# nv-nguyen/gigapose

Hardware: AMD Instinct MI355X
Metric: query-crops/sec (ViT feat + template NN + 4DoF regress), 162 templates, 1/2/4/8 GPU (higher is better)
Workload: dtype f32 (ViT linear layers + attention, matcher, IST convolutions: f32 operands split into f16 hi/lo, 3 x f16 MFMA per k-block, f32 accumulate -- error vs f64 below the f32 fmaf chain's, tests/test_gpu_split.py; everything else f32); 1 GPU; BASELINE configs[1]: dinov2_vitl14 random-init, 1 object(s) x 162 templates, batch=64 crops per GPU, k=5, full path ViT->match->IST->RANSAC->pose; numerics=split, global_batch=64, parallelism=single, streams=single stream, rccl_ranks=0

## Files before the change

gigapose_amd/csrc/gp_match.hip:

```cpp
#include "gp_common.h"

namespace {

__global__ __launch_bounds__(256) void l2norm_cp_kernel(const float* __restrict__ x,
                                                         float* __restrict__ out, int C)
{
    const size_t base = (size_t)blockIdx.x * C * GP_P + threadIdx.x;
    float ss = 0.f;
    for (int c = 0; c < C; ++c) {
        const float v = x[base + (size_t)c * GP_P];
        ss = __builtin_fmaf(v, v, ss);
    }
    const float d = fmaxf(__builtin_sqrtf(ss), 1e-12f);
    const int c0 = blockIdx.y * 32;
    for (int c = c0; c < c0 + 32 && c < C; ++c) out[base + (size_t)c * GP_P] = x[base + (size_t)c * GP_P] / d;
}

using MM = KMajor<4, 2, 2, 4, 16>;
static_assert(MM::BM == 256 && MM::BN == 256 && MM::NT == 512, "matcher tile must be 256x256");

struct alignas(16) MatchSmem {
    float stage[MM::LDS_FLOATS];
    float qmask[GP_P];
    float smask[GP_P];
// ... 471 lines not shown
        sm.smask_p[pidx] = 0.f;
        sm.s_of[pidx] = (short)kDeadPatch;
#pragma unroll
        for (int w = 0; w < 4; ++w) { sm.colv[w][pidx] = 0.f; sm.coli[w][pidx] = 0; }
    }
    __syncthreads();
    int rank = before;
    for (int w = 4 * grp; w < wave; ++w) rank += sm.cnt[w];
    if (live) {
        if (tid < GP_P) {
            sm.t_of[rank] = (short)pidx;
            sm.qmask_p[rank] = mv;
        } else {
            sm.s_of[rank] = (short)pidx;
            sm.smask_p[rank] = mv;
        }
    }
    __syncthreads();
    const int live_t = sm.cnt[0] + sm.cnt[1] + sm.cnt[2] + sm.cnt[3], live_s = sm.cnt[4] + sm.cnt[5] + sm.cnt[6] + sm.cnt[7];
    const int nrb = __builtin_amdgcn_readfirstlane((live_t + 31) >> 5), ncb = __builtin_amdgcn_readfirstlane((live_s + 31) >> 5);
    const MatchWaveTile wt = match_wave_tile_unpack((unsigned)__builtin_amdgcn_readfirstlane((int)kMatchRect[nrb][ncb][wave]));

    const unsigned plane_bytes = (unsigned)GP_P * (unsigned)C * 2u;
    MatchSplitRsrc rs;
    rs.qh = __builtin_amdgcn_make_buffer_rsrc((void*)(q_hi + (size_t)b * GP_P * C), 0, plane_bytes, 0x00020000);
    rs.ql = __builtin_amdgcn_make_buffer_rsrc((void*)(q_lo + (size_t)b * GP_P * C), 0, plane_bytes, 0x00020000);
    rs.bh = __builtin_amdgcn_make_buffer_rsrc((void*)(b_hi + on * GP_P * C), 0, plane_bytes, 0x00020000);
    rs.bl = __builtin_amdgcn_make_buffer_rsrc((void*)((BANK_LO ? b_lo : b_hi) + on * GP_P * C), 0, plane_bytes, 0x00020000);
    {
        const int r0 = tid >> 2, r1 = r0 + 128;
        const unsigned ck = (unsigned)(tid & 3) * 16u, rowb = (unsigned)C * 2u;
        const int t0 = sm.t_of[r0], t1 = sm.t_of[r1], s0 = sm.s_of[r0], s1 = sm.s_of[r1];
        rs.va0 = t0 != kDeadPatch ? (unsigned)t0 * rowb + ck : kMatchOob;
        rs.va1 = t1 != kDeadPatch ? (unsigned)t1 * rowb + ck : kMatchOob;
        rs.vb0 = s0 != kDeadPatch ? (unsigned)s0 * rowb + ck : kMatchOob;
        rs.vb1 = s1 != kDeadPatch ? (unsigned)s1 * rowb + ck : kMatchOob;
    }

    f32x16 acc[2][4];
#pragma unroll
    for (int mi = 0; mi < 2; ++mi)
#pragma unroll
        for (int ni = 0; ni < 4; ++ni)
#pragma unroll
            for (int r = 0; r < 16; ++r) acc[mi][ni][r] = 0.f;
    const int ns = C / MS_BK;
    if (TRACE && tid == 0) trace[1] = wall_clock64();
    if (nrb > 0 && ncb > 0) {
        const int sel = wt.mi_n * 8 + wt.ni_n;
#define M_CASE(MI_, NI_) case MI_ * 8 + NI_: match_split_kloop<BANK_LO, MI_, NI_>(sm, acc, rs, ns, tid, lane, wt.r0, wt.c0, grp); break
        switch (sel) {
            M_CASE(1, 1); M_CASE(1, 2); M_CASE(1, 3); M_CASE(1, 4);
            M_CASE(2, 1); M_CASE(2, 2); M_CASE(2, 3);
            default: match_split_kloop<BANK_LO, 2, 4>(sm, acc, rs, ns, tid, lane, wt.r0, wt.c0, grp); break;
        }
#undef M_CASE
    }
    __syncthreads();
    if (TRACE && tid == 0) trace[2] = wall_clock64();

    constexpr float inv = 1.0f / (kFeatScale * kFeatScale);
#pragma unroll
    for (int mi = 0; mi < 2; ++mi)
#pragma unroll
        for (int ni = 0; ni < 4; ++ni)
#pragma unroll
            for (int r = 0; r < 16; ++r) acc[mi][ni][r] *= inv;
    match_epilogue<true>(sm, acc, b, n, N, thr, patch_thr, idx_t2s, score_t2s, mask_all, sim_avg, trace, src2tar, compact, wt);
}

__global__ __launch_bounds__(256) void l2norm_split_kernel(const float* __restrict__ x, _Float16* __restrict__ hi,
                                                            _Float16* __restrict__ lo, int C, int Cp,
                                                            const float* __restrict__ mask_img = nullptr, int mh = 0, int mw = 0,
                                                            float* __restrict__ patch_mask = nullptr)
{
    __shared__ float t[32][GP_P + 1];
    __shared__ float dn[GP_P];
    const int row = blockIdx.x, p = threadIdx.x;
    if (patch_mask && blockIdx.y == 0)
        patch_mask[(size_t)row * GP_P + p] = mask_img[(size_t)row * mh * mw + (size_t)((p >> 4) * (mh / GP_G)) * mw + (p & 15) * (mw / GP_G)];
    const float* xr = x + (size_t)row * C * GP_P;
    float ss = 0.f;
    int c = 0;
    for (; c + 16 <= C; c += 16) {
        float v[16];
#pragma unroll
        for (int u = 0; u < 16; ++u) v[u] = xr[(size_t)(c + u) * GP_P + p];
#pragma unroll
        for (int u = 0; u < 16; ++u) ss = __builtin_fmaf(v[u], v[u], ss);
    }
    for (; c < C; ++c) {
        const float v = xr[(size_t)c * GP_P + p];
        ss = __builtin_fmaf(v, v, ss);
    }
    dn[p] = fmaxf(__builtin_sqrtf(ss), 1e-12f);
    const int ngrp = Cp / 32, g0 = ngrp * blockIdx.y / gridDim.y, g1 = ngrp * (blockIdx.y + 1) / gridDim.y;
    for (int grp = g0; grp < g1; ++grp) {
        const int c0 = grp * 32;
        __syncthreads();
        for (int r = 0; r < 32; ++r) t[r][p] = (c0 + r < C) ? xr[(size_t)(c0 + r) * GP_P + p] : 0.f;
        __syncthreads();
#pragma unroll
        for (int u = 0; u < 4; ++u) {
            const int item = p + 256 * u, pp = item >> 2, g = item & 3;
            h16x8 h, l;
#pragma unroll
            for (int e = 0; e < 8; ++e) {
                const float v = (t[g * 8 + e][pp] / dn[pp]) * kFeatScale;
                const _Float16 hh = (_Float16)v;
                h[e] = hh;
                l[e] = (_Float16)(v - (float)hh);
            }
            const size_t o = ((size_t)row * GP_P + pp) * Cp + c0 + g * 8;
            *reinterpret_cast<h16x8*>(hi + o) = h;
            *reinterpret_cast<h16x8*>(lo + o) = l;
        }
    }
}

__global__ __launch_bounds__(64) void topk_kernel(const float* __restrict__ sim_avg, int N, int k,
                                                   int* __restrict__ ids, float* __restrict__ scores)
{
    extern __shared__ unsigned char taken[];
    const int b = blockIdx.x, lane = threadIdx.x;
    for (int n = lane; n < N; n += 64) taken[n] = 0;
    __syncthreads();
    const float* v = sim_avg + (size_t)b * N;
    for (int j = 0; j < k; ++j) {
        float bv = 0.f;
        int bi = 0x7fffffff;
        for (int n = lane; n < N; n += 64) {
            if (taken[n]) continue;
            const float x = v[n];
            if (bi == 0x7fffffff || x > bv) { bv = x; bi = n; }
        }
#pragma unroll
        for (int off = 32; off >= 1; off >>= 1) {
            const float ov = __shfl_xor(bv, off);
            const int oi = __shfl_xor(bi, off);
            if (oi != 0x7fffffff && (bi == 0x7fffffff || ov > bv || (ov == bv && oi < bi))) { bv = ov; bi = oi; }
        }
        if (lane == 0) {
            ids[(size_t)b * k + j] = bi;
            scores[(size_t)b * k + j] = bv;
            taken[bi] = 1;
        }
        __syncthreads();
    }
}

__global__ __launch_bounds__(256) void gather_records_kernel(
    const int* __restrict__ ids, const uint8_t* __restrict__ idx_t2s,
    const float* __restrict__ score_t2s, const float* __restrict__ mask_all, int N, int k,
    uint8_t* __restrict__ rec_idx, float* __restrict__ rec_score, float* __restrict__ rec_mask)
{
    const int bk = blockIdx.x, b = bk / k, t = threadIdx.x;
    const size_t src = ((size_t)b * N + ids[bk]) * GP_P + t;
    const size_t dst = (size_t)bk * GP_P + t;
    rec_idx[dst] = idx_t2s[src];
    rec_score[dst] = score_t2s[src];
    rec_mask[dst] = mask_all[src];
}

__global__ __launch_bounds__(256) void format_points_kernel(const uint8_t* __restrict__ rec_idx,
                                                             const float* __restrict__ rec_mask,
                                                             long long* __restrict__ tar_pts,
                                                             long long* __restrict__ src_pts)
{
    const size_t i = (size_t)blockIdx.x * GP_P + threadIdx.x;
    const int t = threadIdx.x;
    const bool valid = rec_mask[i] != 0.f;
    const int js = rec_idx[i];
// ... 215 lines not shown
```

gigapose_amd/csrc/gp_vit.hip:

```cpp
#include "gp_common.h"

int gp_gemm_launch(const float* A, int lda, const float* B, int ldb, float* D, int ldd, int I, int J,
                   int K, int epilogue, const float* bias, const float* scale, const float* res, int ldr,
                   float* sk_ws, hipStream_t st);
int gp_gemm_split_launch(const float* act, int ld_act, const void* whi, const void* wlo, float* D, int ldd, int I, int J,
                         int K, int act_is_b, int epilogue, const float* bias, const float* scale, const float* res, int ldr,
                         hipStream_t st);
bool gp_gemm_split256_usable(int I, int J, int K);
int gp_gemm_split256_launch(const float* act, int ld_act, const void* whi, const void* wlo, float* D, int ldd, int I, int J,
                            int K, int act_is_b, int epilogue, const float* bias, const float* scale, const float* res, int ldr,
                            float* scratch, hipStream_t st);
size_t gp_gemm_streamk_bytes();
int gp_gemm_streamk_reset_launch(float* sk_ws, hipStream_t st);
bool gp_gemm_split256_usable(int I, int J, int K);
bool gp_gemm_planes256_usable(int I, int J, int J_valid, int K);
int gp_gemm_planes256_launch(const void* ahi, const void* alo, const void* bhi, const void* blo, float* D, int ldd, void* ohi,
                             void* olo, int ldo, int I, int J, int J_valid, int K, int epilogue, const float* bias, const float* scale,
                             const float* res, int ldr, float out_scale, float* scratch, hipStream_t st, unsigned long long* trace = nullptr,
                             const GpPlaneOut* po = nullptr);

namespace {

constexpr int PATCH = 14, IMG = 224, KPE = 588, KPE_PAD = 592, T_TOK = 257;

// ... 65 lines not shown

int launch_layernorm(const float* X, float* Y, const float* g, const float* b, int C, int Mpad, float eps,
                     hipStream_t st)
{
    GpProfScope prof(GP_PROF_LN, 8.0 * C * Mpad, st);
    hipLaunchKernelGGL(layernorm_wide_kernel, dim3(Mpad / 64), dim3(1024), 0, st, X, Y, g, b, C, Mpad, eps);
    return 0;
}


typedef _Float16 v16x8 __attribute__((ext_vector_type(8)));
typedef _Float16 v16x4 __attribute__((ext_vector_type(4)));
typedef unsigned int au32x4 __attribute__((ext_vector_type(4)));
typedef float f32x2 __attribute__((ext_vector_type(2)));
constexpr float kPlaneScale = 8.0f;

__global__ __launch_bounds__(1024) void layernorm_planes_kernel(const float* __restrict__ X, _Float16* __restrict__ Yhi,
                                                                 _Float16* __restrict__ Ylo, const float* __restrict__ gamma,
                                                                 const float* __restrict__ beta, int C, int Mpad, float eps,
                                                                 int* __restrict__ status, float plane_scale, float* __restrict__ amax)
{
    __shared__ float red[16][64];
    const int tok = threadIdx.x & 63, sl = threadIdx.x >> 6;
    const int per = C >> 4, c0 = sl * per;
    const float* x = X + (size_t)c0 * Mpad + (size_t)blockIdx.x * 64 + tok;
    int bad = 0;
    float vmax = 0.f;
    float s = 0.f;
#pragma unroll 8
    for (int i = 0; i < per; ++i) s += x[(size_t)i * Mpad];
    red[sl][tok] = s;
    __syncthreads();
    float tot = 0.f;
#pragma unroll
    for (int j = 0; j < 16; ++j) tot += red[j][tok];
    const float mean = tot / (float)C;
    __syncthreads();
    float q = 0.f;
#pragma unroll 8
    for (int i = 0; i < per; ++i) {
        const float d = x[(size_t)i * Mpad] - mean;
        q = __builtin_fmaf(d, d, q);
    }
    red[sl][tok] = q;
    __syncthreads();
    tot = 0.f;
#pragma unroll
    for (int j = 0; j < 16; ++j) tot += red[j][tok];
    const float rstd = 1.0f / __builtin_sqrtf(tot / (float)C + eps);
    __shared__ unsigned int tile[2][128 * 65];
    const float* xb = X + (size_t)blockIdx.x * 64 + tok;
    const int t2 = 8 * (sl & 7) + (tok & 7), g2 = 8 * (sl >> 3) + (tok >> 3);
    const size_t row = ((size_t)blockIdx.x * 64 + t2) * C + 8 * g2;
    const int nchunk = C >> 7;
    for (int k = 0; k < nchunk; ++k) {
        unsigned int* T = tile[k & 1];
#pragma unroll
        for (int e = 0; e < 8; ++e) {
            const int cl = 8 * sl + e, c = 128 * k + cl;
            const float y = (xb[(size_t)c * Mpad] - mean) * rstd * gamma[c] + beta[c];
            const float v = y * plane_scale;
            const _Float16 hh = (_Float16)v;
            const _Float16 ll = (_Float16)(v - (float)hh);
            bad |= !(fabsf(v) <= kSplitPlaneLimit);
            vmax = __builtin_elementwise_maximum(vmax, __builtin_fabsf(v));
            T[cl * 65 + tok] = (unsigned int)__builtin_bit_cast(unsigned short, hh) |
                               ((unsigned int)__builtin_bit_cast(unsigned short, ll) << 16);
        }
        __syncthreads();
        v16x8 h, l;
#pragma unroll
        for (int e = 0; e < 8; ++e) {
            const unsigned int w = T[(8 * g2 + e) * 65 + t2];
            h[e] = __builtin_bit_cast(_Float16, (unsigned short)(w & 0xffffu));
            l[e] = __builtin_bit_cast(_Float16, (unsigned short)(w >> 16));
        }
        *reinterpret_cast<v16x8*>(Yhi + row + 128 * k) = h;
        *reinterpret_cast<v16x8*>(Ylo + row + 128 * k) = l;
    }
    if (bad) gp_raise(status, GP_ST_SPLIT_RANGE);
    if (amax) gp_record_amax(amax, vmax, 1.0f / plane_scale);
}

template <int NK, int TOK = 32>
__global__ __launch_bounds__(512) void layernorm_planes_reg_kernel(const float* __restrict__ X, _Float16* __restrict__ Yhi,
                                                                    _Float16* __restrict__ Ylo, const float* __restrict__ gamma,
                                                                    const float* __restrict__ beta, int Mpad, float eps,
                                                                    int* __restrict__ status, float plane_scale, float* __restrict__ amax)
{
    constexpr int C = 128 * NK, SL = 512 / TOK, CH = 8 * SL, NC = C / CH;
    constexpr int TP = CH + 4;
    static_assert(C % CH == 0 && (TOK == 32 || TOK == 16), "layernorm_planes_reg_kernel: C must be a multiple of the chunk width");
    __shared__ float red[SL][TOK];
    __shared__ __attribute__((aligned(16))) unsigned int tile[2][TOK * TP];
    __shared__ __attribute__((aligned(16))) float gb[2][C];
    const int tok = threadIdx.x & (TOK - 1), sl = threadIdx.x / TOK;
    const size_t tok0 = (size_t)blockIdx.x * TOK;
    float xv[NC][8];
    float s = 0.f;
#pragma unroll
    for (int k = 0; k < NC; ++k)
#pragma unroll
        for (int e = 0; e < 8; ++e) {
            xv[k][e] = X[(size_t)(CH * k + 8 * sl + e) * Mpad + tok0 + tok];
            s += xv[k][e];
        }
    for (int c = threadIdx.x; c < C; c += 512) {
        gb[0][c] = gamma[c];
        gb[1][c] = beta[c];
    }
    red[sl][tok] = s;
    __syncthreads();
    float tot = 0.f;
#pragma unroll
    for (int j = 0; j < SL; ++j) tot += red[j][tok];
    const float mean = tot / (float)C;
    __syncthreads();
    float q = 0.f;
#pragma unroll
    for (int k = 0; k < NC; ++k)
#pragma unroll
        for (int e = 0; e < 8; ++e) {
            const float d = xv[k][e] - mean;
            q = __builtin_fmaf(d, d, q);
        }
    red[sl][tok] = q;
    __syncthreads();
    tot = 0.f;
#pragma unroll
    for (int j = 0; j < SL; ++j) tot += red[j][tok];
    const float rstd = 1.0f / __builtin_sqrtf(tot / (float)C + eps);
    const int g2 = threadIdx.x & (SL - 1), t2 = threadIdx.x / SL;
    const size_t row = (tok0 + t2) * C + 8 * g2;
    int bad = 0;
    float vmax = 0.f;
#pragma unroll
    for (int k = 0; k < NC; ++k) {
        unsigned int* T = tile[k & 1];
        const int c = CH * k + 8 * sl;
        const f32x4 g0 = *reinterpret_cast<const f32x4*>(gb[0] + c), g1 = *reinterpret_cast<const f32x4*>(gb[0] + c + 4);
        const f32x4 b0 = *reinterpret_cast<const f32x4*>(gb[1] + c), b1 = *reinterpret_cast<const f32x4*>(gb[1] + c + 4);
        unsigned int w[8];
#pragma unroll
        for (int e = 0; e < 8; ++e) {
            const float y = (xv[k][e] - mean) * rstd * (e < 4 ? g0[e] : g1[e - 4]) + (e < 4 ? b0[e] : b1[e - 4]);
            const float v = y * plane_scale;
            const _Float16 hh = (_Float16)v;
            const _Float16 ll = (_Float16)(v - (float)hh);
            bad |= !(fabsf(v) <= kSplitPlaneLimit);
            if (amax) vmax = __builtin_elementwise_maximum(vmax, __builtin_fabsf(v));
            w[e] = (unsigned int)__builtin_bit_cast(unsigned short, hh) | ((unsigned int)__builtin_bit_cast(unsigned short, ll) << 16);
        }
        typedef unsigned int u4 __attribute__((ext_vector_type(4)));
        u4 w0 = {w[0], w[1], w[2], w[3]}, w1 = {w[4], w[5], w[6], w[7]};
        *reinterpret_cast<u4*>(T + tok * TP + 8 * sl) = w0;
        *reinterpret_cast<u4*>(T + tok * TP + 8 * sl + 4) = w1;
        __syncthreads();
        const u4 r0 = *reinterpret_cast<const u4*>(T + t2 * TP + 8 * g2), r1 = *reinterpret_cast<const u4*>(T + t2 * TP + 8 * g2 + 4);
        v16x8 h, l;
#pragma unroll
        for (int e = 0; e < 4; ++e) {
            h[e] = __builtin_bit_cast(_Float16, (unsigned short)(r0[e] & 0xffffu));
            l[e] = __builtin_bit_cast(_Float16, (unsigned short)(r0[e] >> 16));
            h[4 + e] = __builtin_bit_cast(_Float16, (unsigned short)(r1[e] & 0xffffu));
            l[4 + e] = __builtin_bit_cast(_Float16, (unsigned short)(r1[e] >> 16));
        }
        *reinterpret_cast<v16x8*>(Yhi + row + CH * k) = h;
        *reinterpret_cast<v16x8*>(Ylo + row + CH * k) = l;
    }
    if (bad) gp_raise(status, GP_ST_SPLIT_RANGE);
    if (amax) gp_record_amax(amax, vmax, 1.0f / plane_scale);
}


static int g_ln_planes_reg = 1;
#ifdef GP_PROBES
extern "C" void gp_vit_set_ln_reg(int on) { g_ln_planes_reg = (on >= 0 && on <= 2) ? on : 1; }
#endif

int launch_layernorm_planes(const float* X, _Float16* hi, _Float16* lo, const float* g, const float* b, int C, int Mpad, float eps,
                            hipStream_t st, float plane_scale = kPlaneScale, float* amax = nullptr)
{
    GpProfScope prof(GP_PROF_LN, 8.0 * C * Mpad, st);
    if (g_ln_planes_reg && C == 1024 && Mpad % 32 == 0 && Mpad / 32 <= 128 && g_ln_planes_reg != 2)
        hipLaunchKernelGGL((layernorm_planes_reg_kernel<8, 16>), dim3(Mpad / 16), dim3(512), 0, st, X, hi, lo, g, b, Mpad, eps, gp_status_buffer(), plane_scale, amax);
    else if (g_ln_planes_reg && C == 1024 && Mpad % 32 == 0)
        hipLaunchKernelGGL(layernorm_planes_reg_kernel<8>, dim3(Mpad / 32), dim3(512), 0, st, X, hi, lo, g, b, Mpad, eps, gp_status_buffer(), plane_scale, amax);
    else if (g_ln_planes_reg && C == 768 && Mpad % 32 == 0)
        hipLaunchKernelGGL(layernorm_planes_reg_kernel<6>, dim3(Mpad / 32), dim3(512), 0, st, X, hi, lo, g, b, Mpad, eps, gp_status_buffer(), plane_scale, amax);
    else
        hipLaunchKernelGGL(layernorm_planes_kernel, dim3(Mpad / 64), dim3(1024), 0, st, X, hi, lo, g, b, C, Mpad, eps, gp_status_buffer(), plane_scale, amax);
    return 0;
}

constexpr int NKT = 9;

__device__ __forceinline__ void attention_body(const float* __restrict__ Qp, const float* __restrict__ Kp,
                                               const float* __restrict__ Vp, float* __restrict__ Op, int q0, int C,
                                               int Mpad, float scale)
{
    const int lane = threadIdx.x, half = lane >> 5, l31 = lane & 31;
    const int tq = q0 + l31;
    const int tq_c = tq < T_TOK ? tq : T_TOK - 1;
    f32x16 o0, o1;
#pragma unroll
    for (int r = 0; r < 16; ++r) { o0[r] = 0.f; o1[r] = 0.f; }
    float m_run = -INFINITY, l_part = 0.f;

#pragma unroll 1
    for (int ch = 0; ch < 3; ++ch) {
        f32x16 s[3];
        int tk_c[3];
#pragma unroll
        for (int t = 0; t < 3; ++t) {
#pragma unroll
            for (int r = 0; r < 16; ++r) s[t][r] = 0.f;
            const int tk = (ch * 3 + t) * 32 + l31;
            tk_c[t] = tk < T_TOK ? tk : T_TOK - 1;
        }
#pragma unroll 8
        for (int kk = 0; kk < 32; ++kk) {
            const size_t drow = (size_t)(2 * kk + half) * Mpad;
            const float qv = Qp[drow + tq_c];
#pragma unroll
            for (int t = 0; t < 3; ++t) {
                const float kv = Kp[drow + tk_c[t]];
                s[t] = __builtin_amdgcn_mfma_f32_32x32x2f32(kv, qv, s[t], 0, 0, 0);
            }
        }
        float cmax = -INFINITY;
#pragma unroll
        for (int t = 0; t < 3; ++t)
#pragma unroll
            for (int r = 0; r < 16; ++r) {
                const int tk = (ch * 3 + t) * 32 + frag_row(r, lane);
                const float v = (tk < T_TOK) ? s[t][r] * scale : -INFINITY;
                s[t][r] = v;
                cmax = fmaxf(cmax, v);
            }
        cmax = fmaxf(cmax, __shfl_xor(cmax, 32));
        const float m_new = fmaxf(m_run, cmax);
        const float alpha = expf(m_run - m_new);
        float psum = 0.f;
#pragma unroll
        for (int t = 0; t < 3; ++t)
#pragma unroll
            for (int r = 0; r < 16; ++r) {
                const float p = expf(s[t][r] - m_new);
                s[t][r] = p;
                psum += p;
            }
        l_part = l_part * alpha + psum;
#pragma unroll
        for (int r = 0; r < 16; ++r) { o0[r] *= alpha; o1[r] *= alpha; }
        m_run = m_new;
#pragma unroll
        for (int t = 0; t < 3; ++t)
#pragma unroll
            for (int r = 0; r < 16; ++r) {
                int tk = (ch * 3 + t) * 32 + frag_row(r, lane);
                tk = tk < T_TOK ? tk : T_TOK - 1;
                const float* vrow = Vp + (size_t)tk * C + l31;
                const float v0 = vrow[0], v1 = vrow[32];
                o0 = __builtin_amdgcn_mfma_f32_32x32x2f32(v0, s[t][r], o0, 0, 0, 0);
                o1 = __builtin_amdgcn_mfma_f32_32x32x2f32(v1, s[t][r], o1, 0, 0, 0);
            }
    }
    const float inv = 1.0f / (l_part + __shfl_xor(l_part, 32));
    if (tq < T_TOK) {
#pragma unroll
        for (int r = 0; r < 16; ++r) {
            const int d = frag_row(r, lane);
// ... 267 lines not shown
            const _Float16* kl = sKl + tid * AKS;
            float a = 0.f;
#pragma unroll
            for (int c8 = 0; c8 < 8; ++c8) {
                const v16x8 h8 = *reinterpret_cast<const v16x8*>(kh + 8 * c8), l8 = *reinterpret_cast<const v16x8*>(kl + 8 * c8);
#pragma unroll
                for (int e = 0; e < 8; ++e) {
                    a = __builtin_fmaf((float)h8[e], xq[8 * c8 + e], a);
                    a = __builtin_fmaf((float)l8[e], xq[8 * c8 + e], a);
                }
            }
            sv = a * (0.125f * inv_s2);
        }
        float mx = sv;
#pragma unroll
        for (int off = 32; off >= 1; off >>= 1) mx = fmaxf(mx, __shfl_xor(mx, off));
        if (lane == 0) xred[0][wave] = mx;
        __syncthreads();
        mx = xred[0][0];
#pragma unroll
        for (int w = 1; w < 8; ++w) mx = fmaxf(mx, xred[0][w]);
        const float pr = tid < T_TOK ? exp_neg(sv - mx) : 0.f;
        if (tid < T_TOK) xs[tid] = pr;
        float ps = pr;
#pragma unroll
        for (int off = 32; off >= 1; off >>= 1) ps += __shfl_xor(ps, off);
        if (lane == 0) xred[1][wave] = ps;
        __syncthreads();
        {
            const _Float16* vh = sVh + lane * AVS + 32 * wave;
            const _Float16* vl = sVl + lane * AVS + 32 * wave;
            v16x4 h4[8], l4[8];
            f32x4 p4[8];
#pragma unroll
            for (int u = 0; u < 8; ++u) {
                h4[u] = *reinterpret_cast<const v16x4*>(vh + 4 * u);
                l4[u] = *reinterpret_cast<const v16x4*>(vl + 4 * u);
                p4[u] = *reinterpret_cast<const f32x4*>(xs + 32 * wave + 4 * u);
            }
            float a = 0.f;
#pragma unroll
            for (int u = 0; u < 8; ++u)
#pragma unroll
                for (int e = 0; e < 4; ++e) {
                    a = __builtin_fmaf((float)h4[u][e], p4[u][e], a);
                    a = __builtin_fmaf((float)l4[u][e], p4[u][e], a);
                }
            if (wave == 0) {
                a = __builtin_fmaf((float)sVh[lane * AVS + T_TOK - 1], xs[T_TOK - 1], a);
                a = __builtin_fmaf((float)sVl[lane * AVS + T_TOK - 1], xs[T_TOK - 1], a);
            }
            xo[wave][lane] = a;
        }
        __syncthreads();
        if (tid < 64) {
            float l = xred[1][0], a = xo[0][tid];
#pragma unroll
            for (int w = 1; w < 8; ++w) { l += xred[1][w]; a += xo[w][tid]; }
            float v = a * (1.0f / l);
            asm volatile("" : "+v"(v));
            const _Float16 hh = (_Float16)v;
            const size_t o = (tok0 + (T_TOK - 1)) * C + h * 64 + tid;
            Ohi[o] = hh;
            Olo[o] = (_Float16)(v - (float)hh);
        }
    }
}

static bool g_vit_planes = true;
#ifdef GP_PROBES
extern "C" void gp_vit_set_planes(int on) { g_vit_planes = on != 0; }
#endif

__global__ __launch_bounds__(256) void features_kernel(const float* __restrict__ X, float* __restrict__ out,
                                                        int C, int Mpad, int normalize, int* __restrict__ status)
{
    const int b = blockIdx.x, p = threadIdx.x;
    const int c0 = (int)((long long)C * blockIdx.y / gridDim.y), c1 = (int)((long long)C * (blockIdx.y + 1) / gridDim.y);
    const float* x = X + (size_t)b * T_TOK + 1 + p;
    float d = 1.f;
    if (normalize) {
        float ss = 0.f;
        int c = 0;
        for (; c + 16 <= C; c += 16) {
            float v[16];
#pragma unroll
            for (int u = 0; u < 16; ++u) v[u] = x[(size_t)(c + u) * Mpad];
#pragma unroll
            for (int u = 0; u < 16; ++u) ss = __builtin_fmaf(v[u], v[u], ss);
        }
        for (; c < C; ++c) {
            const float v = x[(size_t)c * Mpad];
            ss = __builtin_fmaf(v, v, ss);
        }
        d = fmaxf(__builtin_sqrtf(ss), 1e-12f);
        if (blockIdx.y == 0 && !(ss <= 3.0e38f)) gp_raise(status, GP_ST_SPLIT_RANGE);
    }
    float* o = out + (size_t)b * C * GP_P + p;
    for (int c = c0; c < c1; ++c) o[(size_t)c * GP_P] = normalize ? x[(size_t)c * Mpad] / d : x[(size_t)c * Mpad];
}

int launch_features(const float* X, float* out, int B, int C, int Mpad, int normalize, hipStream_t st)
{
    hipLaunchKernelGGL(features_kernel, dim3(B, B >= 64 ? 4 : (B >= 16 ? 16 : 32)), dim3(256), 0, st, X, out, C, Mpad, normalize,
                       gp_status_buffer());
    return 0;
}

inline int round_up(int x, int m) { return (x + m - 1) / m * m; }

}

enum { W_PATCH_WT = 0, W_PATCH_B, W_CLS_POS, W_POS_T, W_HEADER = 4 };
enum { L_LN1_G = 0, L_LN1_B, L_QK_WT, L_QK_B, L_V_WT, L_V_B, L_PROJ_WT, L_PROJ_B, L_LS1, L_LN2_G, L_LN2_B,
       L_FC1_WT, L_FC1_B, L_FC2_WT, L_FC2_B, L_LS2, L_PER_LAYER = 16 };

extern "C" {

size_t gp_vit_workspace_bytes(int B, int dim, int mlp_dim)
{
    if (B <= 0 || dim <= 0 || mlp_dim <= 0) return 0;
    const size_t Mpad = (size_t)round_up(B * T_TOK, 256);
    size_t f = (size_t)mlp_dim * Mpad;
    const size_t pe_need = (size_t)KPE_PAD * B * GP_P + (size_t)dim * B * GP_P;
    if (pe_need > f) f = pe_need;
    return sizeof(float) * ((size_t)5 * dim * Mpad + f) + gp_gemm_streamk_bytes();
}

enum { S_QK_HI = 0, S_QK_LO, S_V_HI, S_V_LO, S_PROJ_HI, S_PROJ_LO, S_FC1_HI, S_FC1_LO, S_FC2_HI, S_FC2_LO, S_PER_LAYER = 10 };
int gp_vit_forward_split2(const float* images, int B, int dim, int depth, int heads, int mlp_dim, float ln_eps,
                          const float* const* weights, int n_weights, const void* const* split, int n_split,
                          float* workspace, size_t workspace_bytes, float* out_features, int normalize,
                          int stop_after_layers, const float* plane_scales, float* plane_amax, void* stream);

int gp_attention_split_scaled(const void* qkv_hi, const void* qkv_lo, void* out_hi, void* out_lo, int B, int heads, int dim, int Mpad,
                              float qkv_scale, void* stream);
int gp_attention_split_scaled(const void* qkv_hi, const void* qkv_lo, void* out_hi, void* out_lo, int B, int heads, int dim, int Mpad,
                              float qkv_scale, void* stream)
{
    GP_REQUIRE(qkv_scale > 0.f, "gp_attention_split: bad plane scale");
    GP_REQUIRE(qkv_hi && qkv_lo && out_hi && out_lo && B > 0 && heads > 0 && dim == heads * 64 && Mpad >= B * T_TOK,
               "gp_attention_split: bad arguments");
    hipLaunchKernelGGL(attention_split_kernel, dim3(xcd_chunked_grid(B * heads)), dim3(ATH), 0, (hipStream_t)stream,
                       (const _Float16*)qkv_hi, (const _Float16*)qkv_lo, (_Float16*)out_hi, (_Float16*)out_lo, B, heads, dim, Mpad, 1.0f / (qkv_scale * qkv_scale));
    GP_CHECK_LAUNCH("gp_attention_split");
    return GP_OK;
}

int gp_layernorm_planes(const float* X, void* out_hi, void* out_lo, const float* gamma, const float* beta, int C, int Mpad, float eps,
                        void* stream)
{
    GP_REQUIRE(X && out_hi && out_lo && gamma && beta && C > 0 && C % 128 == 0 && Mpad > 0 && Mpad % 64 == 0, "gp_layernorm_planes: bad arguments");
    launch_layernorm_planes(X, (_Float16*)out_hi, (_Float16*)out_lo, gamma, beta, C, Mpad, eps, (hipStream_t)stream);
    GP_CHECK_LAUNCH("gp_layernorm_planes");
    return GP_OK;
}

#ifdef GP_PROBES
int gp_vit_attention_f32(const float* qk, const float* vt, float* out, int B, int heads, int dim, int Mpad, void* stream)
{
    GP_REQUIRE(qk && vt && out && B > 0 && heads > 0 && dim == heads * 64 && Mpad > 0 && Mpad % 256 == 0 && (long long)Mpad >= (long long)B * T_TOK,
               "gp_vit_attention_f32: bad arguments");
    launch_attention_f32(qk, vt, out, B, heads, dim, Mpad, (hipStream_t)stream);
    GP_CHECK_LAUNCH("gp_vit_attention_f32");
    return GP_OK;
}

int gp_vit_layernorm_f32(const float* X, float* Y, const float* gamma, const float* beta, int C, int Mpad, float eps, void* stream)
{
    GP_REQUIRE(X && Y && gamma && beta && C > 0 && C % 16 == 0 && Mpad > 0 && Mpad % 64 == 0, "gp_vit_layernorm_f32: bad arguments");
    launch_layernorm(X, Y, gamma, beta, C, Mpad, eps, (hipStream_t)stream);
    GP_CHECK_LAUNCH("gp_vit_layernorm_f32");
    return GP_OK;
}

int gp_vit_features(const float* X, float* out, int B, int C, int Mpad, int normalize, void* stream)
{
    GP_REQUIRE(X && out && B > 0 && C > 0 && Mpad > 0 && (long long)Mpad >= (long long)B * T_TOK, "gp_vit_features: bad arguments");
    launch_features(X, out, B, C, Mpad, normalize, (hipStream_t)stream);
    GP_CHECK_LAUNCH("gp_vit_features");
    return GP_OK;
}
#endif

int gp_vit_forward(const float* images, int B, int dim, int depth, int heads, int mlp_dim, float ln_eps,
                   const float* const* weights, int n_weights, float* workspace, size_t workspace_bytes,
                   float* out_features, int normalize, int stop_after_layers, void* stream)
{
    return gp_vit_forward_split2(images, B, dim, depth, heads, mlp_dim, ln_eps, weights, n_weights, nullptr, 0, workspace,
                                 workspace_bytes, out_features, normalize, stop_after_layers, nullptr, nullptr, stream);
}

int gp_vit_forward_split2(const float* images, int B, int dim, int depth, int heads, int mlp_dim, float ln_eps,
                          const float* const* weights, int n_weights, const void* const* split, int n_split,
                          float* workspace, size_t workspace_bytes, float* out_features, int normalize,
                          int stop_after_layers, const float* plane_scales, float* plane_amax, void* stream)
{
    hipStream_t st = (hipStream_t)stream;
    enum { PS_LN1 = 0, PS_QKV, PS_LN2, PS_GELU, PS_PER_LAYER = 4 };
    if (plane_scales)
        for (int i = 0; i < depth * PS_PER_LAYER; ++i) {
            int ex = 0;
            GP_REQUIRE(plane_scales[i] > 0.f && frexpf(plane_scales[i], &ex) == 0.5f && plane_scales[i] <= 64.f && plane_scales[i] >= 1.0f / 1024.0f,
                       "gp_vit_forward_split2: plane scale %d = %g is not a power of two in [2^-10, 64]", i, (double)plane_scales[i]);
        }
    GP_REQUIRE(B >= 0 && dim > 0 && depth > 0 && heads > 0, "gp_vit_forward: bad config");
    if (B == 0) return GP_OK;
    GP_REQUIRE(dim == heads * 64, "gp_vit_forward: head dim must be 64 (dim=%d heads=%d)", dim, heads);
    GP_REQUIRE(dim % 128 == 0 && mlp_dim % 128 == 0, "gp_vit_forward: dim/mlp_dim must be multiples of 128");
    GP_REQUIRE(n_weights == W_HEADER + depth * L_PER_LAYER, "gp_vit_forward: expected %d weight pointers, got %d",
               W_HEADER + depth * L_PER_LAYER, n_weights);
    GP_REQUIRE(images && weights && workspace && out_features, "gp_vit_forward: null pointer");
    GP_REQUIRE(workspace_bytes >= gp_vit_workspace_bytes(B, dim, mlp_dim), "gp_vit_forward: workspace too small");
    for (int i = 0; i < n_weights; ++i) GP_REQUIRE(weights[i], "gp_vit_forward: weight pointer %d is null", i);
    GP_REQUIRE(split == nullptr || n_split == depth * S_PER_LAYER || n_split == 2 * depth * S_PER_LAYER,
               "gp_vit_forward_split: expected %d (or %d) split planes, got %d", depth * S_PER_LAYER, 2 * depth * S_PER_LAYER, n_split);
    const int sp_stride = (split && n_split == 2 * depth * S_PER_LAYER) ? 2 * S_PER_LAYER : S_PER_LAYER;
    const bool have_x64 = split && sp_stride >= 2 * S_PER_LAYER;
    if (split) {
        GP_REQUIRE(dim % 32 == 0 && mlp_dim % 32 == 0, "gp_vit_forward_split: dim / mlp_dim must be multiples of 32");
        for (int i = 0; i < n_split; ++i) GP_REQUIRE(split[i], "gp_vit_forward_split: split plane %d is null", i);
    }

    const int C = dim, Mpad = round_up(B * T_TOK, 256), BP = B * GP_P;
    float* X = workspace;
    float* Hn = X + (size_t)C * Mpad;
    float* QK = Hn + (size_t)C * Mpad;
    float* Vt = QK + (size_t)2 * C * Mpad;
    float* F = Vt + (size_t)C * Mpad;
    size_t f_floats = (size_t)mlp_dim * Mpad;
    if ((size_t)KPE_PAD * B * GP_P + (size_t)dim * B * GP_P > f_floats) f_floats = (size_t)KPE_PAD * B * GP_P + (size_t)dim * B * GP_P;
    float* SK = F + f_floats;
    float* col = F;
    float* pe = F + (size_t)KPE_PAD * BP;
    int rc;

    if ((rc = gp_gemm_streamk_reset_launch(SK, st))) return rc;
    hipLaunchKernelGGL(im2col_kernel, dim3(KPE_PAD, B), dim3(256), 0, st, images, col, B);
    GP_CHECK_LAUNCH("gp_vit_forward/im2col");
    if ((rc = gp_gemm_launch(weights[W_PATCH_WT], C, col, BP, pe, BP, C, BP, KPE_PAD, 1 ,
                             weights[W_PATCH_B], nullptr, nullptr, 0, SK, st)))
        return rc;
    hipLaunchKernelGGL(embed_kernel, dim3(C, B + 1), dim3(320), 0, st, pe, weights[W_CLS_POS], weights[W_POS_T],
                       X, B, Mpad);
    GP_CHECK_LAUNCH("gp_vit_forward/embed");

    const int nl = (stop_after_layers >= 0 && stop_after_layers < depth) ? stop_after_layers : depth;
    const int Mtok = B * T_TOK;
    const bool planes = have_x64 && g_vit_planes && gp_gemm_planes256_usable(2 * C, Mpad, Mtok, C) &&
                        gp_gemm_planes256_usable(C, Mpad, Mtok, C) && gp_gemm_planes256_usable(mlp_dim, Mpad, Mtok, C) &&
                        gp_gemm_planes256_usable(C, Mpad, Mtok, mlp_dim);
    if (planes) {
        _Float16* Hhi = reinterpret_cast<_Float16*>(Hn);
        _Float16* Hlo = Hhi + (size_t)C * Mpad;
        _Float16* Fhi = reinterpret_cast<_Float16*>(F);
        _Float16* Flo = Fhi + (size_t)mlp_dim * Mpad;
        const float ps_default[PS_PER_LAYER] = {kPlaneScale, kPlaneScale, kPlaneScale, kPlaneScale};
        for (int l = 0; l < nl; ++l) {
            const float* const* w = weights + W_HEADER + l * L_PER_LAYER;
            const void* const* sq = split + l * sp_stride + S_PER_LAYER;
            const float* ps = plane_scales ? plane_scales + l * PS_PER_LAYER : ps_default;
            float* am = plane_amax ? plane_amax + l * PS_PER_LAYER : nullptr;
            const float os_ln1 = 1.0f / (ps[PS_LN1] * 64.0f), os_qkv = 1.0f / (ps[PS_QKV] * 64.0f), os_ln2 = 1.0f / (ps[PS_LN2] * 64.0f),
                        os_gelu = 1.0f / (ps[PS_GELU] * 64.0f);
            const GpPlaneOut po_qkv{ps[PS_QKV], am ? am + PS_QKV : nullptr}, po_gelu{ps[PS_GELU], am ? am + PS_GELU : nullptr};
            launch_layernorm_planes(X, Hhi, Hlo, w[L_LN1_G], w[L_LN1_B], C, Mpad, ln_eps, st, ps[PS_LN1], am ? am + PS_LN1 : nullptr);
            GP_CHECK_LAUNCH("gp_vit_forward/layernorm_planes");
            _Float16* Ahi = reinterpret_cast<_Float16*>(QK);
            _Float16* Alo = Ahi + (size_t)3 * C * Mpad;
            const bool fused_qkv = (const char*)sq[S_V_HI] == (const char*)sq[S_QK_HI] + (size_t)2 * C * C * 2 &&
                                   (const char*)sq[S_V_LO] == (const char*)sq[S_QK_LO] + (size_t)2 * C * C * 2 && w[L_V_B] == w[L_QK_B] + 2 * C &&
                                   gp_gemm_planes256_usable(3 * C, Mpad, Mtok, C);
            if (fused_qkv) {
                if ((rc = gp_gemm_planes256_launch(sq[S_QK_HI], sq[S_QK_LO], Hhi, Hlo, nullptr, 0, Ahi, Alo, 3 * C, 3 * C, Mpad, Mtok, C,
                                                   7 , w[L_QK_B], nullptr, nullptr, 0, os_ln1, SK, st, nullptr, &po_qkv)))
                    return rc;
            } else {
                if ((rc = gp_gemm_planes256_launch(sq[S_QK_HI], sq[S_QK_LO], Hhi, Hlo, nullptr, 0, Ahi, Alo, 3 * C, 2 * C, Mpad, Mtok, C,
                                                   7 , w[L_QK_B], nullptr, nullptr, 0, os_ln1, SK, st, nullptr, &po_qkv)))
                    return rc;
                if ((rc = gp_gemm_planes256_launch(sq[S_V_HI], sq[S_V_LO], Hhi, Hlo, nullptr, 0, Ahi + 2 * C, Alo + 2 * C, 3 * C, C, Mpad, Mtok, C,
                                                   7 , w[L_V_B], nullptr, nullptr, 0, os_ln1, SK, st, nullptr, &po_qkv)))
                    return rc;
            }
            {
                GpProfScope prof(GP_PROF_ATTN, 4.0 * B * heads * 257.0 * 257.0 * 64.0, st);
                hipLaunchKernelGGL(attention_split_kernel, dim3(xcd_chunked_grid(B * heads)), dim3(ATH), 0, st, Ahi, Alo, Hhi, Hlo, B,
                                   heads, C, Mpad, 1.0f / (ps[PS_QKV] * ps[PS_QKV]));
            }
            GP_CHECK_LAUNCH("gp_vit_forward/attention_split");
            if ((rc = gp_gemm_planes256_launch(sq[S_PROJ_HI], sq[S_PROJ_LO], Hhi, Hlo, X, Mpad, nullptr, nullptr, 0, C, Mpad, Mtok, C,
                                               3 , w[L_PROJ_B], w[L_LS1], X, Mpad, os_qkv, SK, st)))
                return rc;
            launch_layernorm_planes(X, Hhi, Hlo, w[L_LN2_G], w[L_LN2_B], C, Mpad, ln_eps, st, ps[PS_LN2], am ? am + PS_LN2 : nullptr);
            GP_CHECK_LAUNCH("gp_vit_forward/layernorm_planes");
            if ((rc = gp_gemm_planes256_launch(sq[S_FC1_HI], sq[S_FC1_LO], Hhi, Hlo, nullptr, 0, Fhi, Flo, mlp_dim, mlp_dim, Mpad, Mtok, C,
                                               6 , w[L_FC1_B], nullptr, nullptr, 0, os_ln2, SK, st, nullptr, &po_gelu)))
                return rc;
            if ((rc = gp_gemm_planes256_launch(sq[S_FC2_HI], sq[S_FC2_LO], Fhi, Flo, X, Mpad, nullptr, nullptr, 0, C, Mpad, Mtok, mlp_dim,
                                               3 , w[L_FC2_B], w[L_LS2], X, Mpad, os_gelu, SK, st)))
                return rc;
        }
    }
    for (int l = planes ? nl : 0; l < nl; ++l) {
        const float* const* w = weights + W_HEADER + l * L_PER_LAYER;
        launch_layernorm(X, Hn, w[L_LN1_G], w[L_LN1_B], C, Mpad, ln_eps, st);
        GP_CHECK_LAUNCH("gp_vit_forward/layernorm");
        const void* const* sp = split ? split + l * sp_stride : nullptr;
        const void* const* sq = (sp && have_x64) ? sp + S_PER_LAYER : nullptr;
        auto sgemm = [&](const float* act, int ld_act, int which, float* D, int ldd, int I, int J, int K, int act_is_b, int epi,
                         const float* bias, const float* scale, const float* res, int ldr) -> int {
            if (sq && gp_gemm_split256_usable(I, J, K))
                return gp_gemm_split256_launch(act, ld_act, sq[which], sq[which + 1], D, ldd, I, J, K, act_is_b, epi, bias, scale, res,
                                               ldr, SK, st);
            return gp_gemm_split_launch(act, ld_act, sp[which], sp[which + 1], D, ldd, I, J, K, act_is_b, epi, bias, scale, res, ldr, st);
        };
        if (sp) rc = sgemm(Hn, Mpad, S_QK_HI, QK, Mpad, 2 * C, Mpad, C, 1, 1, w[L_QK_B], nullptr, nullptr, 0);
        else rc = gp_gemm_launch(w[L_QK_WT], 2 * C, Hn, Mpad, QK, Mpad, 2 * C, Mpad, C, 1, w[L_QK_B], nullptr, nullptr, 0, SK, st);
        if (rc) return rc;
        if (sp) rc = sgemm(Hn, Mpad, S_V_HI, Vt, C, Mpad, C, C, 0, 4 , w[L_V_B], nullptr, nullptr, 0);
        else rc = gp_gemm_launch(Hn, Mpad, w[L_V_WT], C, Vt, C, Mpad, C, C, 4 , w[L_V_B], nullptr, nullptr, 0, SK, st);
        if (rc) return rc;
        launch_attention_f32(QK, Vt, Hn, B, heads, C, Mpad, st);
        GP_CHECK_LAUNCH("gp_vit_forward/attention");
        if (sp) rc = sgemm(Hn, Mpad, S_PROJ_HI, X, Mpad, C, Mpad, C, 1, 3, w[L_PROJ_B], w[L_LS1], X, Mpad);
        else rc = gp_gemm_launch(w[L_PROJ_WT], C, Hn, Mpad, X, Mpad, C, Mpad, C, 3, w[L_PROJ_B], w[L_LS1], X, Mpad, SK, st);
        if (rc) return rc;
        launch_layernorm(X, Hn, w[L_LN2_G], w[L_LN2_B], C, Mpad, ln_eps, st);
        GP_CHECK_LAUNCH("gp_vit_forward/layernorm");
        if (sp) rc = sgemm(Hn, Mpad, S_FC1_HI, F, Mpad, mlp_dim, Mpad, C, 1, 2 , w[L_FC1_B], nullptr, nullptr, 0);
        else rc = gp_gemm_launch(w[L_FC1_WT], mlp_dim, Hn, Mpad, F, Mpad, mlp_dim, Mpad, C, 2 , w[L_FC1_B], nullptr,
                                 nullptr, 0, SK, st);
        if (rc) return rc;
        if (sp) rc = sgemm(F, Mpad, S_FC2_HI, X, Mpad, C, Mpad, mlp_dim, 1, 3, w[L_FC2_B], w[L_LS2], X, Mpad);
        else rc = gp_gemm_launch(w[L_FC2_WT], C, F, Mpad, X, Mpad, C, Mpad, mlp_dim, 3, w[L_FC2_B], w[L_LS2], X, Mpad, SK, st);
        if (rc) return rc;
    }
    launch_features(X, out_features, B, C, Mpad, normalize, st);
    GP_CHECK_LAUNCH("gp_vit_forward/features");
    return GP_OK;
}

}
```

Before: 1574 query-crops/sec.

## Layernorm only valid token rows, folding leftover tokens into resident blocks

After: 1584 query-crops/sec, median of 6. About the same (+0.6%).

```diff
diff --git a/gigapose_amd/csrc/gp_match.hip b/gigapose_amd/csrc/gp_match.hip
--- a/gigapose_amd/csrc/gp_match.hip
+++ b/gigapose_amd/csrc/gp_match.hip
@@ -577,12 +577,13 @@
     const float* xr = x + (size_t)row * C * GP_P;
     float ss = 0.f;
     int c = 0;
-    for (; c + 16 <= C; c += 16) {
-        float v[16];
-#pragma unroll
-        for (int u = 0; u < 16; ++u) v[u] = xr[(size_t)(c + u) * GP_P + p];
-#pragma unroll
-        for (int u = 0; u < 16; ++u) ss = __builtin_fmaf(v[u], v[u], ss);
+    constexpr int NL = 64;
+    for (; c + NL <= C; c += NL) {
+        float v[NL];
+#pragma unroll
+        for (int u = 0; u < NL; ++u) v[u] = xr[(size_t)(c + u) * GP_P + p];
+#pragma unroll
+        for (int u = 0; u < NL; ++u) ss = __builtin_fmaf(v[u], v[u], ss);
     }
     for (; c < C; ++c) {
         const float v = xr[(size_t)c * GP_P + p];
diff --git a/gigapose_amd/csrc/gp_vit.hip b/gigapose_amd/csrc/gp_vit.hip
--- a/gigapose_amd/csrc/gp_vit.hip
+++ b/gigapose_amd/csrc/gp_vit.hip
@@ -171,15 +171,26 @@
     if (amax) gp_record_amax(amax, vmax, 1.0f / plane_scale);
 }
 
-template <int NK, int TOK = 32>
+template <int NK, int TOK = 32, bool XT = false>
 __global__ __launch_bounds__(512) void layernorm_planes_reg_kernel(const float* __restrict__ X, _Float16* __restrict__ Yhi,
                                                                     _Float16* __restrict__ Ylo, const float* __restrict__ gamma,
                                                                     const float* __restrict__ beta, int Mpad, float eps,
-                                                                    int* __restrict__ status, float plane_scale, float* __restrict__ amax)
+                                                                    int* __restrict__ status, float plane_scale, float* __restrict__ amax,
+                                                                    int nx)
 {
     constexpr int C = 128 * NK, SL = 512 / TOK, CH = 8 * SL, NC = C / CH;
     constexpr int TP = CH + 4;
     static_assert(C % CH == 0 && (TOK == 32 || TOK == 16), "layernorm_planes_reg_kernel: C must be a multiple of the chunk width");
+    static_assert(!XT || (TOK == 32 && C % 512 == 0), "layernorm_planes_reg_kernel: the extra token is staged by 512 threads, C / 512 values each");
+    constexpr int XE = XT ? C / 512 : 1;
+    __shared__ __attribute__((aligned(16))) float xs[XT ? C : 4];
+    __shared__ float xred[2][SL];
+    const bool has_x = XT && (int)blockIdx.x < nx;
+    const size_t xcol = (size_t)gridDim.x * TOK + blockIdx.x;
+    float xe[XE];
+    if (has_x)
+#pragma unroll
+        for (int j = 0; j < XE; ++j) xe[j] = X[(size_t)(threadIdx.x + 512 * j) * Mpad + xcol];
     __shared__ float red[SL][TOK];
     __shared__ __attribute__((aligned(16))) unsigned int tile[2][TOK * TP];
     __shared__ __attribute__((aligned(16))) float gb[2][C];
@@ -199,11 +210,24 @@
         gb[1][c] = beta[c];
     }
     red[sl][tok] = s;
+    if (has_x)
+#pragma unroll
+        for (int j = 0; j < XE; ++j) xs[threadIdx.x + 512 * j] = xe[j];
     __syncthreads();
     float tot = 0.f;
 #pragma unroll
     for (int j = 0; j < SL; ++j) tot += red[j][tok];
     const float mean = tot / (float)C;
+    if (has_x && threadIdx.x < SL) {
+        float sx = 0.f;
+#pragma unroll
+        for (int k = 0; k < NC; ++k) {
+            const f32x4 v0 = *reinterpret_cast<const f32x4*>(xs + CH * k + 8 * threadIdx.x), v1 = *reinterpret_cast<const f32x4*>(xs + CH * k + 8 * threadIdx.x + 4);
+#pragma unroll
+            for (int e = 0; e < 8; ++e) sx += e < 4 ? v0[e] : v1[e - 4];
+        }
+        xred[0][threadIdx.x] = sx;
+    }
     __syncthreads();
     float q = 0.f;
 #pragma unroll
@@ -214,6 +238,27 @@
             q = __builtin_fmaf(d, d, q);
         }
     red[sl][tok] = q;
+    const bool x_conv = has_x && threadIdx.x < C / 8;
+    float mean_x = 0.f;
+    if (x_conv) {
+        float totx = 0.f;
+#pragma unroll
+        for (int j = 0; j < SL; ++j) totx += xred[0][j];
+        mean_x = totx / (float)C;
+        if (threadIdx.x < SL) {
+            float qx = 0.f;
+#pragma unroll
+            for (int k = 0; k < NC; ++k) {
+                const f32x4 v0 = *reinterpret_cast<const f32x4*>(xs + CH * k + 8 * threadIdx.x), v1 = *reinterpret_cast<const f32x4*>(xs + CH * k + 8 * threadIdx.x + 4);
+#pragma unroll
+                for (int e = 0; e < 8; ++e) {
+                    const float d = (e < 4 ? v0[e] : v1[e - 4]) - mean_x;
+                    qx = __builtin_fmaf(d, d, qx);
+                }
+            }
+            xred[1][threadIdx.x] = qx;
+        }
+    }
     __syncthreads();
     tot = 0.f;
 #pragma unroll
@@ -223,6 +268,29 @@
     const size_t row = (tok0 + t2) * C + 8 * g2;
     int bad = 0;
     float vmax = 0.f;
+    if (x_conv) {
+        float totx = 0.f;
+#pragma unroll
+        for (int j = 0; j < SL; ++j) totx += xred[1][j];
+        const float rstd_x = 1.0f / __builtin_sqrtf(totx / (float)C + eps);
+        const int c = 8 * threadIdx.x;
+        const f32x4 x0 = *reinterpret_cast<const f32x4*>(xs + c), x1 = *reinterpret_cast<const f32x4*>(xs + c + 4);
+        const f32x4 g0 = *reinterpret_cast<const f32x4*>(gb[0] + c), g1 = *reinterpret_cast<const f32x4*>(gb[0] + c + 4);
+        const f32x4 b0 = *reinterpret_cast<const f32x4*>(gb[1] + c), b1 = *reinterpret_cast<const f32x4*>(gb[1] + c + 4);
+        v16x8 h, l;
+#pragma unroll
+        for (int e = 0; e < 8; ++e) {
+            const float y = ((e < 4 ? x0[e] : x1[e - 4]) - mean_x) * rstd_x * (e < 4 ? g0[e] : g1[e - 4]) + (e < 4 ? b0[e] : b1[e - 4]);
+            const float v = y * plane_scale;
+            const _Float16 hh = (_Float16)v;
+            bad |= !(fabsf(v) <= kSplitPlaneLimit);
+            if (amax) vmax = __builtin_elementwise_maximum(vmax, __builtin_fabsf(v));
+            h[e] = hh;
+            l[e] = (_Float16)(v - (float)hh);
+        }
+        *reinterpret_cast<v16x8*>(Yhi + xcol * C + c) = h;
+        *reinterpret_cast<v16x8*>(Ylo + xcol * C + c) = l;
+    }
 #pragma unroll
     for (int k = 0; k < NC; ++k) {
         unsigned int* T = tile[k & 1];
@@ -264,19 +332,43 @@
 
 static int g_ln_planes_reg = 1;
 #ifdef GP_PROBES
-extern "C" void gp_vit_set_ln_reg(int on) { g_ln_planes_reg = (on >= 0 && on <= 2) ? on : 1; }
+extern "C" void gp_vit_set_ln_reg(int on) { g_ln_planes_reg = ((on >= 0 && on <= 2) || (on >= 16 && on <= 65536)) ? on : 1; }
 #endif
 
+static int ln_resident_blocks()
+{
+    static int cached[64];
+    int dev = 0, cu = 0;
+    if (hipGetDevice(&dev) != hipSuccess || dev < 0) return 0;
+    if (dev < 64 && cached[dev]) return cached[dev];
+    if (hipDeviceGetAttribute(&cu, hipDeviceAttributeMultiprocessorCount, dev) != hipSuccess || cu <= 0) return 0;
+    if (dev < 64) cached[dev] = 2 * cu;
+    return 2 * cu;
+}
+
+static long long ln_extra_token_blocks(int C, int rows)
+{
+    const int mode = g_ln_planes_reg;
+    const long long R = mode >= 16 ? mode : (mode == 1 ? ln_resident_blocks() : 0);
+    return (C == 1024 && rows % 32 == 0 && R > 0 && rows > 32 * R && rows - 32 * R <= R) ? R : 0;
+}
+
 int launch_layernorm_planes(const float* X, _Float16* hi, _Float16* lo, const float* g, const float* b, int C, int Mpad, float eps,
-                            hipStream_t st, float plane_scale = kPlaneScale, float* amax = nullptr)
+                            hipStream_t st, float plane_scale = kPlaneScale, float* amax = nullptr, int rows = 0)
 {
     GpProfScope prof(GP_PROF_LN, 8.0 * C * Mpad, st);
-    if (g_ln_planes_reg && C == 1024 && Mpad % 32 == 0 && Mpad / 32 <= 128 && g_ln_planes_reg != 2)
-        hipLaunchKernelGGL((layernorm_planes_reg_kernel<8, 16>), dim3(Mpad / 16), dim3(512), 0, st, X, hi, lo, g, b, Mpad, eps, gp_status_buffer(), plane_scale, amax);
-    else if (g_ln_planes_reg && C == 1024 && Mpad % 32 == 0)
-        hipLaunchKernelGGL(layernorm_planes_reg_kernel<8>, dim3(Mpad / 32), dim3(512), 0, st, X, hi, lo, g, b, Mpad, eps, gp_status_buffer(), plane_scale, amax);
-    else if (g_ln_planes_reg && C == 768 && Mpad % 32 == 0)
-        hipLaunchKernelGGL(layernorm_planes_reg_kernel<6>, dim3(Mpad / 32), dim3(512), 0, st, X, hi, lo, g, b, Mpad, eps, gp_status_buffer(), plane_scale, amax);
+    const int mode = g_ln_planes_reg;
+    if (rows <= 0 || rows > Mpad || rows % 32 || mode == 2) rows = Mpad;
+    const long long R = ln_extra_token_blocks(C, rows);
+    if (R > 0 && Mpad % 32 == 0)
+        hipLaunchKernelGGL((layernorm_planes_reg_kernel<8, 32, true>), dim3((unsigned)R), dim3(512), 0, st, X, hi, lo, g, b, Mpad, eps, gp_status_buffer(), plane_scale, amax,
+                           (int)(rows - 32 * R));
+    else if (mode == 1 && C == 1024 && Mpad % 32 == 0 && Mpad / 32 <= 128)
+        hipLaunchKernelGGL((layernorm_planes_reg_kernel<8, 16>), dim3(rows / 16), dim3(512), 0, st, X, hi, lo, g, b, Mpad, eps, gp_status_buffer(), plane_scale, amax, 0);
+    else if (mode && C == 1024 && Mpad % 32 == 0)
+        hipLaunchKernelGGL(layernorm_planes_reg_kernel<8>, dim3(rows / 32), dim3(512), 0, st, X, hi, lo, g, b, Mpad, eps, gp_status_buffer(), plane_scale, amax, 0);
+    else if (mode && C == 768 && Mpad % 32 == 0)
+        hipLaunchKernelGGL(layernorm_planes_reg_kernel<6>, dim3(rows / 32), dim3(512), 0, st, X, hi, lo, g, b, Mpad, eps, gp_status_buffer(), plane_scale, amax, 0);
     else
         hipLaunchKernelGGL(layernorm_planes_kernel, dim3(Mpad / 64), dim3(1024), 0, st, X, hi, lo, g, b, C, Mpad, eps, gp_status_buffer(), plane_scale, amax);
     return 0;
@@ -710,12 +802,13 @@
     if (normalize) {
         float ss = 0.f;
         int c = 0;
-        for (; c + 16 <= C; c += 16) {
-            float v[16];
-#pragma unroll
-            for (int u = 0; u < 16; ++u) v[u] = x[(size_t)(c + u) * Mpad];
-#pragma unroll
-            for (int u = 0; u < 16; ++u) ss = __builtin_fmaf(v[u], v[u], ss);
+        constexpr int NL = 64;
+        for (; c + NL <= C; c += NL) {
+            float v[NL];
+#pragma unroll
+            for (int u = 0; u < NL; ++u) v[u] = x[(size_t)(c + u) * Mpad];
+#pragma unroll
+            for (int u = 0; u < NL; ++u) ss = __builtin_fmaf(v[u], v[u], ss);
         }
         for (; c < C; ++c) {
             const float v = x[(size_t)c * Mpad];
@@ -725,7 +818,15 @@
         if (blockIdx.y == 0 && !(ss <= 3.0e38f)) gp_raise(status, GP_ST_SPLIT_RANGE);
     }
     float* o = out + (size_t)b * C * GP_P + p;
-    for (int c = c0; c < c1; ++c) o[(size_t)c * GP_P] = normalize ? x[(size_t)c * Mpad] / d : x[(size_t)c * Mpad];
+    int c = c0;
+    for (; c + 16 <= c1; c += 16) {
+        float v[16];
+#pragma unroll
+        for (int u = 0; u < 16; ++u) v[u] = x[(size_t)(c + u) * Mpad];
+#pragma unroll
+        for (int u = 0; u < 16; ++u) o[(size_t)(c + u) * GP_P] = normalize ? v[u] / d : v[u];
+    }
+    for (; c < c1; ++c) o[(size_t)c * GP_P] = normalize ? x[(size_t)c * Mpad] / d : x[(size_t)c * Mpad];
 }
 
 int launch_features(const float* X, float* out, int B, int C, int Mpad, int normalize, hipStream_t st)
@@ -778,7 +879,9 @@
 int gp_layernorm_planes(const float* X, void* out_hi, void* out_lo, const float* gamma, const float* beta, int C, int Mpad, float eps,
                         void* stream)
 {
-    GP_REQUIRE(X && out_hi && out_lo && gamma && beta && C > 0 && C % 128 == 0 && Mpad > 0 && Mpad % 64 == 0, "gp_layernorm_planes: bad arguments");
+    GP_REQUIRE(X && out_hi && out_lo && gamma && beta && C > 0 && C % 128 == 0 && Mpad > 0 &&
+                   (Mpad % 64 == 0 || ln_extra_token_blocks(C, Mpad) > 0 || (g_ln_planes_reg == 2 && C == 1024 && Mpad % 32 == 0)),
+               "gp_layernorm_planes: bad arguments");
     launch_layernorm_planes(X, (_Float16*)out_hi, (_Float16*)out_lo, gamma, beta, C, Mpad, eps, (hipStream_t)stream);
     GP_CHECK_LAUNCH("gp_layernorm_planes");
     return GP_OK;
@@ -884,6 +987,7 @@
         _Float16* Fhi = reinterpret_cast<_Float16*>(F);
         _Float16* Flo = Fhi + (size_t)mlp_dim * Mpad;
         const float ps_default[PS_PER_LAYER] = {kPlaneScale, kPlaneScale, kPlaneScale, kPlaneScale};
+        const int ln_rows = min(Mpad, round_up(Mtok, 32));
         for (int l = 0; l < nl; ++l) {
             const float* const* w = weights + W_HEADER + l * L_PER_LAYER;
             const void* const* sq = split + l * sp_stride + S_PER_LAYER;
@@ -892,7 +996,7 @@
             const float os_ln1 = 1.0f / (ps[PS_LN1] * 64.0f), os_qkv = 1.0f / (ps[PS_QKV] * 64.0f), os_ln2 = 1.0f / (ps[PS_LN2] * 64.0f),
                         os_gelu = 1.0f / (ps[PS_GELU] * 64.0f);
             const GpPlaneOut po_qkv{ps[PS_QKV], am ? am + PS_QKV : nullptr}, po_gelu{ps[PS_GELU], am ? am + PS_GELU : nullptr};
-            launch_layernorm_planes(X, Hhi, Hlo, w[L_LN1_G], w[L_LN1_B], C, Mpad, ln_eps, st, ps[PS_LN1], am ? am + PS_LN1 : nullptr);
+            launch_layernorm_planes(X, Hhi, Hlo, w[L_LN1_G], w[L_LN1_B], C, Mpad, ln_eps, st, ps[PS_LN1], am ? am + PS_LN1 : nullptr, ln_rows);
             GP_CHECK_LAUNCH("gp_vit_forward/layernorm_planes");
             _Float16* Ahi = reinterpret_cast<_Float16*>(QK);
             _Float16* Alo = Ahi + (size_t)3 * C * Mpad;
@@ -920,7 +1024,7 @@
             if ((rc = gp_gemm_planes256_launch(sq[S_PROJ_HI], sq[S_PROJ_LO], Hhi, Hlo, X, Mpad, nullptr, nullptr, 0, C, Mpad, Mtok, C,
                                                3 , w[L_PROJ_B], w[L_LS1], X, Mpad, os_qkv, SK, st)))
                 return rc;
-            launch_layernorm_planes(X, Hhi, Hlo, w[L_LN2_G], w[L_LN2_B], C, Mpad, ln_eps, st, ps[PS_LN2], am ? am + PS_LN2 : nullptr);
+            launch_layernorm_planes(X, Hhi, Hlo, w[L_LN2_G], w[L_LN2_B], C, Mpad, ln_eps, st, ps[PS_LN2], am ? am + PS_LN2 : nullptr, ln_rows);
             GP_CHECK_LAUNCH("gp_vit_forward/layernorm_planes");
             if ((rc = gp_gemm_planes256_launch(sq[S_FC1_HI], sq[S_FC1_LO], Hhi, Hlo, nullptr, 0, Fhi, Flo, mlp_dim, mlp_dim, Mpad, Mtok, C,
                                                6 , w[L_FC1_B], nullptr, nullptr, 0, os_ln2, SK, st, nullptr, &po_gelu)))
```
